# rlvc/FEALESS

Hardware: AMD Instinct MI355X
Metric: frames/sec (640x480 RGB-D x N templates, 20 ICP iters) (higher is better)
Workload: dtype u8

## Files before the change

fealess_amd/csrc/fl_context.hip:

```cpp
#include "fl_internal.h"
#include <stdlib.h>
#include <stdarg.h>
#include <string.h>
#include <algorithm>

int fl_set_error(fl_context *ctx, int code, const char *fmt, ...)
{
  if (ctx) {
    va_list ap;
    va_start(ap, fmt);
    vsnprintf(ctx->err, sizeof(ctx->err), fmt, ap);
    va_end(ap);
  }
  return code;
}

int fl_scratch(fl_context *ctx, size_t bytes, void **out)
{
  if (int rc = fl_context_join(ctx)) return rc;
  if (bytes > ctx->scratch_bytes) {
    if (ctx->scratch) {
      FL_HIP(ctx, hipStreamSynchronize(ctx->stream));
      FL_HIP(ctx, hipFree(ctx->scratch));
      ctx->scratch = nullptr;
      ctx->scratch_bytes = 0;
    }
    size_t nb = fl_align(bytes + bytes / 4, 1 << 20);
    FL_HIP(ctx, hipMalloc(&ctx->scratch, nb));
    ctx->scratch_bytes = nb;
  }
  *out = ctx->scratch;
  return FL_OK;
}

int fl_pinned(fl_context *ctx, size_t bytes, void **out)
{
  if (int rc = fl_context_join(ctx)) return rc;
  if (bytes > ctx->pinned_bytes) {
    if (ctx->pinned) {
      FL_HIP(ctx, hipStreamSynchronize(ctx->stream));
      FL_HIP(ctx, hipHostFree(ctx->pinned));
      ctx->pinned = nullptr;
      ctx->pinned_bytes = 0;
    }
    size_t nb = fl_align(bytes, 1 << 16);
    FL_HIP(ctx, hipHostMalloc(&ctx->pinned, nb, hipHostMallocDefault));
    ctx->pinned_bytes = nb;
  }
  *out = ctx->pinned;
  return FL_OK;
}

int fl_context_join(fl_context *ctx)
{
  if (!ctx->icp_pending) return FL_OK;
  ctx->icp_pending = false;
  FL_HIP(ctx, hipStreamWaitEvent(ctx->stream, ctx->ev_icp_tail, 0));
  return FL_OK;
}

int fl_context_sync_all(fl_context *ctx)
{
  FL_HIP(ctx, hipStreamSynchronize(ctx->stream));
  if (ctx->icp_stream) FL_HIP(ctx, hipStreamSynchronize(ctx->icp_stream));
  ctx->icp_pending = false;
  return FL_OK;
}

int fl_icp_stream(fl_context *ctx, hipStream_t *out)
{
  const long mode = ctx->opt.pipeline_icp;
  if (ctx->icp_stream && ctx->icp_stream_mode != mode) {
    FL_HIP(ctx, hipStreamSynchronize(ctx->icp_stream));
    FL_HIP(ctx, hipStreamDestroy(ctx->icp_stream));
    ctx->icp_stream = nullptr;
  }
  if (!ctx->icp_stream) {
    int least = 0, greatest = 0;
    FL_HIP(ctx, hipDeviceGetStreamPriorityRange(&least, &greatest));
    FL_HIP(ctx, hipStreamCreateWithPriority(&ctx->icp_stream, hipStreamNonBlocking, mode == 2 ? greatest : (mode == 3 ? least : 0)));
    ctx->icp_stream_mode = mode;
  }
  if (!ctx->ev_icp_tail) FL_HIP(ctx, hipEventCreateWithFlags(&ctx->ev_icp_tail, hipEventDisableTiming));
  *out = ctx->icp_stream;
  return FL_OK;
}

extern "C" int fl_abi_version(void) { return FL_ABI_VERSION; }

struct FlOptionName { const char *name, *env; long fl_context::Options::*field; bool hex; long lo, hi; };
static const FlOptionName fl_option_names[] = {
  {"scan_prune", "FL_SCAN_PRUNE", &fl_context::Options::scan_prune, false, 0, 1},
  {"scan_prune_mid", "FL_SCAN_PRUNE_MID", &fl_context::Options::scan_prune_mid, true, -1, 0xFF},
  {"scan_prune_lanes", "FL_SCAN_PRUNE_LANES", &fl_context::Options::scan_prune_lanes, false, 0, 1},
  {"scan_prune_step", "FL_SCAN_PRUNE_STEP", &fl_context::Options::scan_prune_step, false, 0, 8},
  {"scan_first", "FL_SCAN_FIRST", &fl_context::Options::scan_first, false, 0, 16},
  {"icp_wide", "FL_ICP_WIDE", &fl_context::Options::icp_wide, false, -1, 1},
  {"icp_occ", "FL_ICP_OCC", &fl_context::Options::icp_occ, false, 0, 5},
  {"icp_idx16", "FL_ICP_IDX16", &fl_context::Options::icp_idx16, false, -1, 1},
  {"icp_order", "FL_ICP_ORDER", &fl_context::Options::icp_order, false, 0, 1},
  {"icp_wg_per_cu", "FL_ICP_WG_PER_CU", &fl_context::Options::icp_wg_per_cu, false, 0, 3},
  {"eager_frontend", "FL_EAGER_FRONTEND", &fl_context::Options::eager_frontend, false, 0, 1},
  {"dev_poison", "FL_DEV_POISON", &fl_context::Options::dev_poison, false, 0, 1},
  {"ws_pad", "FL_DEV_WS_PAD", &fl_context::Options::ws_pad, false, 0, 16l << 20},
  {"pipeline_icp", "FL_PIPELINE_ICP", &fl_context::Options::pipeline_icp, false, 0, 3},
  {"frontend_chunk_rows", "FL_FRONTEND_CHUNK_ROWS", &fl_context::Options::frontend_chunk_rows, false, 0, 60 * 1024},
  {"scan_run", "FL_SCAN_RUN", &fl_context::Options::scan_run, false, 0, 64},
  {"refine_lds", "FL_REFINE_LDS", &fl_context::Options::refine_lds, false, 0, 2},
  {"refine_lds_bytes", "FL_REFINE_LDS_BYTES", &fl_context::Options::refine_lds_bytes, false, 0, FL_REFINE_LDS_BYTES},
  {"verify_fused", "FL_VERIFY_FUSED", &fl_context::Options::verify_fused, false, 0, 1},
  {"verify_fused_px", "FL_VERIFY_FUSED_PX", &fl_context::Options::verify_fused_px, false, 0, FL_VERIFY_FUSED_PX},
};

static bool fl_option_valid(const FlOptionName &o, long v)
{
  if (v < o.lo || v > o.hi) return false;
  if (o.field == &fl_context::Options::frontend_chunk_rows) return v % 60 == 0;
  if (o.field == &fl_context::Options::verify_fused_px) return v == 0 || v >= FL_WAVE;
  if (o.field == &fl_context::Options::scan_prune_step) return v == 0 || v == 2 || v == 4 || v == 8;
  if (o.field == &fl_context::Options::scan_first) return v == 0 || v == 8 || v == 12 || v == 14 || v == 16;
  return o.field != &fl_context::Options::icp_occ || v == 0 || v >= 4;
}

extern "C" int fl_context_create(int device, fl_context **out)
{
  if (!out) return FL_ERR_INVALID;
  *out = nullptr;
  int n = 0;
  if (hipGetDeviceCount(&n) != hipSuccess || n <= 0) return FL_ERR_NO_DEVICE;
  if (device < 0 || device >= n) return FL_ERR_INVALID;
  fl_context *ctx = new fl_context();
  ctx->device = device;
  if (hipSetDevice(device) != hipSuccess ||
      hipStreamCreateWithFlags(&ctx->own_stream, hipStreamNonBlocking) != hipSuccess) {
    delete ctx;
    return FL_ERR_HIP;
  }
  ctx->stream = ctx->own_stream;
  {
    hipDeviceProp_t prop;
    if (hipGetDeviceProperties(&prop, device) == hipSuccess && prop.multiProcessorCount > 0) ctx->cus = prop.multiProcessorCount;
  }
  for (const FlOptionName &o : fl_option_names)
    if (const char *e = getenv(o.env)) {
      const long v = o.hex ? (long)strtoul(e, nullptr, 16) : atol(e);
      if (fl_option_valid(o, v)) ctx->opt.*(o.field) = v;
    }
  *out = ctx;
  return FL_OK;
}

extern "C" void *fl_context_get_stream(fl_context *ctx) { return ctx ? (void *)ctx->stream : nullptr; }
extern "C" int fl_context_get_device(const fl_context *ctx) { return ctx ? ctx->device : -1; }
extern "C" fl_context *fl_detector_get_context(fl_detector *det) { return det ? det->ctx : nullptr; }

extern "C" int fl_context_set_option(fl_context *ctx, const char *name, long value)
{
  if (!ctx || !name) return FL_ERR_INVALID;
  for (const FlOptionName &o : fl_option_names)
    if (!strcmp(name, o.name)) {
      if (!fl_option_valid(o, value)) return fl_set_error(ctx, FL_ERR_INVALID, "option '%s': %ld is out of range", name, value);
      ctx->opt.*(o.field) = value;
      return FL_OK;
    }
  return fl_set_error(ctx, FL_ERR_INVALID, "unknown option '%s'", name);
}

extern "C" int fl_context_get_option(const fl_context *ctx, const char *name, long *value)
{
  if (!ctx || !name || !value) return FL_ERR_INVALID;
  for (const FlOptionName &o : fl_option_names)
    if (!strcmp(name, o.name)) { *value = ctx->opt.*(o.field); return FL_OK; }
  return FL_ERR_INVALID;
}

static void context_release(fl_context *ctx)
{
  if (ctx->device < 0) { delete ctx; return; }
  (void)hipSetDevice(ctx->device);
  (void)fl_context_sync_all(ctx);
  if (ctx->icp_stream) (void)hipStreamDestroy(ctx->icp_stream);
  if (ctx->ev_icp_tail) (void)hipEventDestroy(ctx->ev_icp_tail);
  if (ctx->scratch) (void)hipFree(ctx->scratch);
  if (ctx->pinned) (void)hipHostFree(ctx->pinned);
  if (ctx->own_stream) (void)hipStreamDestroy(ctx->own_stream);
  delete ctx;
}

extern "C" void fl_context_destroy(fl_context *ctx)
{
  if (!ctx) return;
  if (ctx->detectors > 0) { ctx->destroy_pending = true; return; }
  context_release(ctx);
}

extern "C" const char *fl_last_error(const fl_context *ctx) { return ctx ? ctx->err : "null context"; }

extern "C" int fl_context_set_stream(fl_context *ctx, void *hip_stream)
{
  if (!ctx) return FL_ERR_INVALID;
  if (int rc = fl_context_sync_all(ctx)) return rc;
  ctx->stream = hip_stream ? (hipStream_t)hip_stream : ctx->own_stream;
  return FL_OK;
}

extern "C" int fl_context_synchronize(fl_context *ctx)
{
  if (!ctx) return FL_ERR_INVALID;
  FL_HIP(ctx, hipSetDevice(ctx->device));
  return fl_context_sync_all(ctx);
}

extern "C" size_t fl_lm_label_stride(int w, int h, int T)
{
  size_t W = (size_t)(w / T), H = (size_t)(h / T);
  size_t pad = W * H + 16 * W + 64;
  size_t s = (size_t)T * T * W * H + pad;
  return (s + 63) & ~(size_t)63;
}

extern "C" int fl_detector_create(fl_context *ctx, int modalities, int levels, const int *T_at_level,
                                  fl_detector **out)
{
  if (!ctx || !out || !T_at_level) return FL_ERR_INVALID;
  if (modalities < 1 || modalities > FL_MAX_MODALITIES || levels < 1 || levels > FL_MAX_LEVELS)
    return fl_set_error(ctx, FL_ERR_INVALID, "modalities must be 1..%d and levels 1..%d", FL_MAX_MODALITIES,
                        FL_MAX_LEVELS);
  for (int l = 0; l < levels; ++l)
    if (T_at_level[l] < 1 || T_at_level[l] > 16) return fl_set_error(ctx, FL_ERR_INVALID, "T out of range");
  fl_detector *det = new fl_detector();
  det->ctx = ctx;
  ++ctx->detectors;
  det->M = modalities;
  det->L = levels;
  for (int l = 0; l < levels; ++l) det->T[l] = T_at_level[l];
  memset(&det->times, 0, sizeof(det->times));
  *out = det;
  return FL_OK;
}

static void free_device_tables(fl_detector *det)
{
  (void)hipFree(det->d_scan_items);
  (void)hipFree(det->d_scan_off);
  (void)hipFree(det->d_fine_hdr);
  (void)hipFree(det->d_fine_box);
  (void)hipFree(det->d_fine_feat);
  (void)hipFree(det->d_pyr);
  (void)hipFree(det->d_poses);
  (void)hipFree(det->d_class_first);
  (void)hipFree(det->d_item_enabled);
  (void)hipFree((void *)det->d_depth_ptrs);
  (void)hipFree(det->d_ws);
  (void)hipFree(det->d_results);
  if (det->h_results) (void)hipHostFree(det->h_results);
  det->d_scan_items = nullptr;
  det->n_scan_items = 0;
  det->scan_item_g.clear();
  det->d_scan_off = nullptr;
  det->d_fine_hdr = nullptr;
  det->d_fine_box = nullptr;
  det->d_fine_feat = nullptr;
  det->d_pyr = nullptr;
  det->d_poses = nullptr;
// ... 486 lines not shown
```

fealess_amd/csrc/fl_frontend.hip:

```cpp
#include "fl_internal.h"
#include <float.h>
#include <type_traits>

#ifndef FL_CQ_DOT4
#define FL_CQ_DOT4 1
#endif

__device__ __forceinline__ int clampi(int v, int lo, int hi) { return v < lo ? lo : (v > hi ? hi : v); }
__device__ __forceinline__ int reflect101(int p, int len)
{
  if (len == 1) return 0;
  while (p < 0 || p >= len) p = p < 0 ? -p : 2 * len - 2 - p;
  return p;
}

__device__ __forceinline__ float fast_atan2_deg(float y, float x)
{
  const float p1 = 0.9997878412794807f * (float)(180 / 3.14159265358979323846);
  const float p3 = -0.3258083974640975f * (float)(180 / 3.14159265358979323846);
  const float p5 = 0.1555786518463281f * (float)(180 / 3.14159265358979323846);
  const float p7 = -0.04432655554792128f * (float)(180 / 3.14159265358979323846);
  const float ax = fabsf(x), ay = fabsf(y);
  const bool steep = !(ax >= ay);
  const float c = (steep ? ax : ay) / ((steep ? ay : ax) + (float)DBL_EPSILON);
  const float c2 = c * c;
  const float poly = (((p7 * c2 + p5) * c2 + p3) * c2 + p1) * c;
  float a = steep ? 90.f - poly : poly;
  if (x < 0) a = 180.f - a;
  if (y < 0) a = 360.f - a;
  return a;
}

#define CQ_COLS 60
#define CQ_CH 60

__device__ __forceinline__ unsigned wave_from_prev(unsigned v) { return (unsigned)__builtin_amdgcn_update_dpp((int)v, (int)v, 0x138, 0xF, 0xF, false); }
__device__ __forceinline__ unsigned wave_from_next(unsigned v) { return (unsigned)__builtin_amdgcn_update_dpp((int)v, (int)v, 0x130, 0xF, 0xF, false); }
__device__ __forceinline__ unsigned wave_from_prev0(unsigned v) { return (unsigned)__builtin_amdgcn_update_dpp(0, (int)v, 0x138, 0xF, 0xF, true); }
__device__ __forceinline__ unsigned wave_from_next0(unsigned v) { return (unsigned)__builtin_amdgcn_update_dpp(0, (int)v, 0x130, 0xF, 0xF, true); }

__host__ __device__ __forceinline__ void cq_window_addr(uint32_t row_mis, int w, int xc, uint32_t *off, uint32_t *shift, int *first)
{
  const int f = xc - 3 < 0 ? 0 : (xc - 3 > w - 7 ? w - 7 : xc - 3);
  const uint32_t o = row_mis + 3u * (uint32_t)f;
  *off = o & ~3u;
  *shift = o & 3u;
  *first = f;
}

__host__ __device__ __forceinline__ uint32_t cq_alignbyte(uint32_t hi, uint32_t lo, uint32_t s)
{
#if defined(__HIP_DEVICE_COMPILE__)
  return __builtin_amdgcn_alignbyte(hi, lo, s);
#else
  return (uint32_t)((((uint64_t)hi << 32) | lo) >> (8 * (s & 3u)));
#endif
}

__host__ __device__ __forceinline__ void cq_window(const uint8_t *__restrict__ row4, uint32_t row_mis, int w, int xc, bool any_left,
                                                   bool any_right, uint32_t *wd)
{
  uint32_t off, shift;
  int first;
  cq_window_addr(row_mis, w, xc, &off, &shift, &first);
  const int dpx = xc - 3 - first;
  uint32_t d[6];
  const uint8_t *q = (const uint8_t *)__builtin_assume_aligned(row4 + off, 4);
  __builtin_memcpy(d, q, 16);
  __builtin_memcpy(d + 4, q + 16, 8);
#pragma unroll
  for (int k = 0; k < 5; ++k) wd[k] = cq_alignbyte(d[k + 1], d[k], shift);
  wd[5] = cq_alignbyte(d[5], d[5], shift);
#define CQ_TAKE(e0, e1, e2, e3, e4, e5, e6, e7, e8)                                                                                 \
  {                                                                                                                                 \
    const bool b0 = (dw & 1u) != 0u, b1 = (dw & 2u) != 0u;                                                                          \
    const uint32_t t0 = b0 ? e1 : e0, t1 = b0 ? e2 : e1, t2 = b0 ? e3 : e2, t3 = b0 ? e4 : e3, t4 = b0 ? e5 : e4, t5 = b0 ? e6 : e5, \
                   t6 = b0 ? e7 : e6, t7 = b0 ? e8 : e7;                                                                            \
    const uint32_t g0 = b1 ? t2 : t0, g1 = b1 ? t3 : t1, g2 = b1 ? t4 : t2, g3 = b1 ? t5 : t3, g4 = b1 ? t6 : t4, g5 = b1 ? t7 : t5; \
    wd[0] = cq_alignbyte(g1, g0, s);                                                                                                \
    wd[1] = cq_alignbyte(g2, g1, s);                                                                                                \
    wd[2] = cq_alignbyte(g3, g2, s);                                                                                                \
    wd[3] = cq_alignbyte(g4, g3, s);                                                                                                \
    wd[4] = cq_alignbyte(g5, g4, s);                                                                                                \
    wd[5] = cq_alignbyte(g5, g5, s);                                                                                                \
  }
  if (any_left) {
    const uint32_t s = dpx < 0 ? (uint32_t)-dpx : 0u, dw = 3u - s;
    const uint32_t p = wd[0] & 0xFFFFFFu;
    CQ_TAKE((p | (p << 24)), ((p >> 8) | (p << 16)), ((p >> 16) | (p << 8)), wd[0], wd[1], wd[2], wd[3], wd[4], wd[5])
  }
  if (any_right) {
    const uint32_t n = dpx > 0 ? 3u * (uint32_t)dpx : 0u, dw = n >> 2, s = n & 3u;
    const uint32_t p = (wd[4] >> 16) | ((wd[5] & 0xFFu) << 16);
    CQ_TAKE(wd[0], wd[1], wd[2], wd[3], wd[4], ((p >> 16) | (p << 8)), (p | (p << 24)), ((p >> 8) | (p << 16)), 0u)
  }
#undef CQ_TAKE
}

template <bool kNarrow>
__device__ __forceinline__ void cq_hrow(const uint8_t *__restrict__ src, int w, int h, int row, int xc, bool any_left, bool any_right,
                                        int *h3)
{
  const int kk[7] = {8, 28, 56, 72, 56, 28, 8};
  const uint8_t *p = src + (size_t)clampi(row, 0, h - 1) * (size_t)(w * 3);
  int a0 = 0, a1 = 0, a2 = 0;
  if (!kNarrow) {
    const uint32_t mis = (uint32_t)(uintptr_t)p & 3u;
    uint32_t wd[6];
    cq_window(p - mis, mis, w, xc, any_left, any_right, wd);
#if FL_CQ_DOT4
    unsigned acc[3] = {0u, 0u, 0u};
#pragma unroll
    for (int ch = 0; ch < 3; ++ch)
#pragma unroll
      for (int k = 0; k < 6; ++k) {
        unsigned wk = 0;
#pragma unroll
        for (int t = 0; t < 7; ++t)
          if (((3 * t + ch) >> 2) == k) wk |= (unsigned)kk[t] << (8 * ((3 * t + ch) & 3));
        if (wk != 0u) acc[ch] = __builtin_amdgcn_udot4(wd[k], wk, acc[ch], false);
      }
    a0 = (int)acc[0]; a1 = (int)acc[1]; a2 = (int)acc[2];
#else
#pragma unroll
    for (int t = 0; t < 7; ++t) {
      const int b0 = 3 * t, b1 = 3 * t + 1, b2 = 3 * t + 2;
      a0 += kk[t] * (int)((wd[b0 >> 2] >> (8 * (b0 & 3))) & 0xFFu);
      a1 += kk[t] * (int)((wd[b1 >> 2] >> (8 * (b1 & 3))) & 0xFFu);
      a2 += kk[t] * (int)((wd[b2 >> 2] >> (8 * (b2 & 3))) & 0xFFu);
    }
#endif
  } else {
#pragma unroll
    for (int t = 0; t < 7; ++t) {
      const uint8_t *q = p + 3 * clampi(xc + t - 3, 0, w - 1);
      a0 += kk[t] * q[0];
      a1 += kk[t] * q[1];
      a2 += kk[t] * q[2];
    }
  }
  h3[0] = a0;
  h3[1] = a1;
  h3[2] = a2;
}

extern "C" void fl_dev_cq_window_addr(unsigned row_mis, int w, int xc, unsigned *off, unsigned *shift, int *first)
{
  cq_window_addr(row_mis, w, xc, off, shift, first);
}
extern "C" void fl_dev_cq_window_taps(const uint8_t *row4, unsigned row_mis, int w, int xc, int any_left, int any_right, uint8_t *taps21)
{
  uint32_t wd[6];
  cq_window(row4, row_mis, w, xc, any_left != 0, any_right != 0, wd);
  for (int b = 0; b < 21; ++b) taps21[b] = (uint8_t)(wd[b >> 2] >> (8 * (b & 3)));
}

#ifndef FL_CQ_WPE
#define FL_CQ_WPE 6
#endif
template <bool kMag, bool kNarrow>
__global__ __launch_bounds__(256) __attribute__((amdgpu_waves_per_eu(kNarrow ? 6 : FL_CQ_WPE, kNarrow ? 6 : FL_CQ_WPE))) void k_color_quantize(const uint8_t *__restrict__ bgr, size_t in_stride,
                                                        uint8_t *__restrict__ dst, size_t out_stride, int w, int h,
                                                        float threshold_sq, int nstrips, int nchunks, int chunk_rows,
                                                        float *__restrict__ mag_out, const uint32_t *__restrict__ tiles,
                                                        size_t tiles_stride)
{
  const int wave = __builtin_amdgcn_readfirstlane((int)(threadIdx.x >> 6)), lane = threadIdx.x & 63;
  const int item = blockIdx.x * 4 + wave;
  if (item >= nstrips * nchunks) return;
  const int strip = item % nstrips, chunk = item / nstrips;
  int row_lo = 0, row_hi = h - 1;
  if (tiles) {
    const uint32_t *tb = tiles + (size_t)blockIdx.z * tiles_stride;
    const int t = chunk * nstrips + strip;
    if (!((tb[FL_TILE_WORDS + (t >> 5)] >> (t & 31)) & 1u)) return;
    const uint32_t rw = tb[2 * FL_TILE_WORDS + 32 * FL_TILE_WORDS + t];
    row_lo = (int)(rw >> 16);
    row_hi = (int)(rw & 0xFFFFu);
  }
  const uint8_t *src = bgr + (size_t)blockIdx.z * in_stride;
  uint8_t *out = dst + (size_t)blockIdx.z * out_stride;
  const int x = strip * CQ_COLS + lane - 2;
  const int xc = clampi(x, 0, w - 1);
  const int y0 = max(chunk * chunk_rows, row_lo), y1 = min(min(h, chunk * chunk_rows + chunk_rows), row_hi + 1);
  if (y0 >= y1) return;
  const bool any_left = strip == 0, any_right = strip * CQ_COLS + 61 > w - 4;

  int H[7][3];
  {
    const int center = clampi(y0 - 2, 0, h - 1);
#pragma unroll
    for (int i = 0; i < 7; ++i) cq_hrow<kNarrow>(src, w, h, center + i - 3, xc, any_left, any_right, H[i]);
  }
  uint32_t Sl[3] = {0, 0, 0}, Sc[3] = {0, 0, 0}, Sr[3] = {0, 0, 0};
  uint32_t Qp[3] = {0, 0, 0};
  float Mg[3] = {0.f, 0.f, 0.f};
  auto smooth = [&](int p) __attribute__((always_inline)) {
    uint32_t vv[3];
#pragma unroll
    for (int ch = 0; ch < 3; ++ch)
      vv[ch] = __umul24(8u, (unsigned)(H[p % 7][ch] + H[(p + 6) % 7][ch])) + __umul24(28u, (unsigned)(H[(p + 1) % 7][ch] + H[(p + 5) % 7][ch])) +
               __umul24(56u, (unsigned)(H[(p + 2) % 7][ch] + H[(p + 4) % 7][ch])) + __umul24(72u, (unsigned)H[(p + 3) % 7][ch]);
    const uint32_t S = (uint32_t)(((int)vv[0] + (1 << 15)) >> 16) | ((uint32_t)(((int)vv[1] + (1 << 15)) >> 16) << 8) |
                       ((uint32_t)(((int)vv[2] + (1 << 15)) >> 16) << 16);
    const uint32_t L = wave_from_prev0(S), R = wave_from_next0(S);
    Sl[0] = Sl[1]; Sl[1] = Sl[2]; Sl[2] = L;
    Sc[0] = Sc[1]; Sc[1] = Sc[2]; Sc[2] = S;
    Sr[0] = Sr[1]; Sr[1] = Sr[2]; Sr[2] = R;
  };
  auto again = [&]() __attribute__((always_inline)) {
    Sl[0] = Sl[1]; Sl[1] = Sl[2];
    Sc[0] = Sc[1]; Sc[1] = Sc[2];
    Sr[0] = Sr[1]; Sr[1] = Sr[2];
  };
  auto finish = [&](int yv) __attribute__((always_inline)) {
    if (yv < y0) return;
    const int ys = yv - 1;
    int bdx = 0, bdy = 0, bmag = 0;
    {
      int dxs[3], dys[3], mags[3];
#pragma unroll
      for (int ch = 0; ch < 3; ++ch) {
        const int sh = 8 * ch;
#define PX(v) ((int)(((v) >> sh) & 0xFFu))
        const int dx = (PX(Sr[0]) - PX(Sl[0])) + 2 * (PX(Sr[1]) - PX(Sl[1])) + (PX(Sr[2]) - PX(Sl[2]));
        const int dy = (PX(Sl[2]) - PX(Sl[0])) + 2 * (PX(Sc[2]) - PX(Sc[0])) + (PX(Sr[2]) - PX(Sr[0]));
#undef PX
        dxs[ch] = dx;
        dys[ch] = dy;
        mags[ch] = __mul24(dx, dx) + __mul24(dy, dy);
      }
      if (mags[0] >= mags[1] && mags[0] >= mags[2]) { bdx = dxs[0]; bdy = dys[0]; bmag = mags[0]; }
      else if (mags[1] >= mags[0] && mags[1] >= mags[2]) { bdx = dxs[1]; bdy = dys[1]; bmag = mags[1]; }
      else { bdx = dxs[2]; bdy = dys[2]; bmag = mags[2]; }
    }
    const float ang = fast_atan2_deg((float)bdy, (float)bdx);
    int qi = __float2int_rn(ang * (float)(16.0 / 360.0));
    qi = qi < 0 ? 0 : (qi > 255 ? 255 : qi);
    const bool inside = ys > 0 && ys < h - 1 && x > 0 && x < w - 1;
    const uint32_t q = inside ? (uint32_t)(qi & 7) : 0u;
    const uint32_t oh = 1u << (4 * q);
    const uint32_t ohl = wave_from_prev0(oh), ohr = wave_from_next0(oh);
    Qp[0] = Qp[1]; Qp[1] = Qp[2]; Qp[2] = oh + ohl + ohr;
    Mg[0] = Mg[1]; Mg[1] = Mg[2]; Mg[2] = (float)bmag;
    if (yv < y0 + 2) return;
    const int yo = yv - 2;
    if (lane >= 2 && lane < 2 + CQ_COLS && x < w && yo < y1) {
      uint8_t res = 0;
      if (yo >= 1 && yo < h - 1 && x >= 1 && x < w - 1 && Mg[1] > threshold_sq) {
        const unsigned hist = Qp[0] + Qp[1] + Qp[2];
        const unsigned maj = (hist + 0x33333333u) & 0x88888888u;
        if (maj) res = (uint8_t)(1u << ((__ffs((int)maj) - 4) >> 2));
      }
      out[(size_t)yo * w + x] = res;
      if (kMag) mag_out[(size_t)blockIdx.z * out_stride + (size_t)yo * w + x] = Mg[1];
      else if (mag_out) mag_out[(size_t)yo * w + x] = Mg[1];
    }
  };

  const int ylast = y1 + 1, yadv = min(ylast, h - 1);
  int yv = y0 - 2;
  smooth(0);
  for (++yv; yv <= min(ylast, 0); ++yv) {
    again();
    finish(yv);
  }
  for (;;) {
#pragma unroll
    for (int P = 0; P < 7; ++P) {
      if (yv > yadv) goto below;
      cq_hrow<kNarrow>(src, w, h, yv + 3, xc, any_left, any_right, H[P]);
      smooth(P + 1);
      finish(yv);
      ++yv;
    }
  }
below:
  for (; yv <= ylast; ++yv) {
    again();
    finish(yv);
  }
}

int fl_launch_quantized_orientations(fl_context *ctx, const uint8_t *bgr, size_t in_stride, uint8_t *dst,
                                     size_t out_stride, int n_frames, int w, int h, float weak_threshold)
{
  return fl_launch_quantized_orientations_mag(ctx, bgr, in_stride, dst, out_stride, n_frames, w, h, weak_threshold, nullptr);
}

#define FL_CHUNK_FILL 4
template <typename K>
static long waves_per_cu(K kernel, long *cache)
{
  if (*cache == 0) {
    int blocks = 0;
    *cache = hipOccupancyMaxActiveBlocksPerMultiprocessor(&blocks, kernel, 256, 0) == hipSuccess && blocks > 0 ? 4l * blocks : 32;
  }
  return *cache;
}
static int fl_eager_chunk_rows(const fl_context *ctx, long per_cu, int nstrips, int n_frames, int h)
{
  if (ctx->opt.frontend_chunk_rows) return (int)ctx->opt.frontend_chunk_rows;
  const long need = (long)FL_CHUNK_FILL * ctx->cus * per_cu;
  return h > 60 && (long)nstrips * n_frames * ((h + 119) / 120) >= need ? 120 : 60;
}

static_assert(CQ_COLS == FL_TILE && CQ_CH == FL_TILE, "the lazy tile grid is k_color_quantize's work decomposition");
static int launch_color_quantize(fl_context *ctx, const uint8_t *bgr, size_t in_stride, uint8_t *dst, size_t out_stride, int n_frames,
                                 int w, int h, float weak_threshold, float *mag_out, const uint32_t *tiles, size_t tiles_stride)
{
  static long per_cu[4] = {0, 0, 0, 0};
  const int nstrips = (w + CQ_COLS - 1) / CQ_COLS;
  const bool narrow = w < 8;
  auto launch = [&](auto kernel, long *cache) {
    const int rows = tiles ? CQ_CH : fl_eager_chunk_rows(ctx, waves_per_cu(kernel, cache), nstrips, n_frames, h);
    const int nchunks = (h + rows - 1) / rows;
    dim3 grid((nstrips * nchunks + 3) / 4, 1, n_frames);
    hipLaunchKernelGGL(kernel, grid, dim3(256), 0, ctx->stream, bgr, in_stride, dst, out_stride, w, h, weak_threshold * weak_threshold,
                       nstrips, nchunks, rows, mag_out, tiles, tiles_stride);
  };
  if (mag_out) {
    if (narrow) launch(k_color_quantize<true, true>, &per_cu[3]);
    else launch(k_color_quantize<true, false>, &per_cu[1]);
  } else {
    if (narrow) launch(k_color_quantize<false, true>, &per_cu[2]);
    else launch(k_color_quantize<false, false>, &per_cu[0]);
  }
  FL_HIP(ctx, hipGetLastError());
  return FL_OK;
}

int fl_launch_quantized_orientations_mag(fl_context *ctx, const uint8_t *bgr, size_t in_stride, uint8_t *dst,
                                         size_t out_stride, int n_frames, int w, int h, float weak_threshold, float *mag_out)
{
  return launch_color_quantize(ctx, bgr, in_stride, dst, out_stride, n_frames, w, h, weak_threshold, mag_out, nullptr, 0);
}

__device__ __forceinline__ void pyrdown_general_px(const uint8_t *__restrict__ src, int w, int h, int x, int y, uint8_t *o)
{
  const int k[5] = {1, 4, 6, 4, 1};
  int acc0 = 0, acc1 = 0, acc2 = 0;
#pragma unroll
  for (int j = 0; j < 5; ++j) {
    const int yy = reflect101(2 * y + j - 2, h);
    int r0 = 0, r1 = 0, r2 = 0;
#pragma unroll
    for (int i = 0; i < 5; ++i) {
      const int xx = reflect101(2 * x + i - 2, w);
      const uint8_t *p = src + ((size_t)yy * w + xx) * 3;
      r0 += k[i] * p[0];
      r1 += k[i] * p[1];
      r2 += k[i] * p[2];
    }
    acc0 += k[j] * r0;
    acc1 += k[j] * r1;
    acc2 += k[j] * r2;
  }
  o[0] = (uint8_t)((acc0 + 128) >> 8);
  o[1] = (uint8_t)((acc1 + 128) >> 8);
  o[2] = (uint8_t)((acc2 + 128) >> 8);
}

__global__ __launch_bounds__(256) void k_pyrdown_general(const uint8_t *__restrict__ src_, size_t in_stride,
                                                         uint8_t *__restrict__ dst_, size_t out_stride, int w, int h)
{
  const int dw = w / 2, dh = h / 2;
  const int x = blockIdx.x * 32 + (threadIdx.x & 31), y = blockIdx.y * 8 + (threadIdx.x >> 5);
  if (x >= dw || y >= dh) return;
  const uint8_t *src = src_ + (size_t)blockIdx.z * in_stride;
  uint8_t *dst = dst_ + (size_t)blockIdx.z * out_stride;
  pyrdown_general_px(src, w, h, x, y, dst + ((size_t)y * dw + x) * 3);
}

#define PD_ROWS 8
__global__ __launch_bounds__(256) void k_pyrdown_pairs(const uint8_t *__restrict__ src_, size_t in_stride,
                                                       uint8_t *__restrict__ dst_, size_t out_stride, int w, int h)
{
  const int dw = w / 2, dh = h / 2, np = dw / 2;
  const int per = (np + (int)gridDim.x - 1) / (int)gridDim.x, lane = threadIdx.x & 63;
  const int xp = blockIdx.x * per + lane;
  const int y0 = (blockIdx.y * 4 + (threadIdx.x >> 6)) * PD_ROWS;
  if (lane >= per || xp >= np || y0 >= dh) return;
  const uint8_t *src = src_ + (size_t)blockIdx.z * in_stride;
  uint8_t *dst = dst_ + (size_t)blockIdx.z * out_stride;
  const bool first = xp == 0, last = xp == np - 1;
  const bool wave_first = blockIdx.x == 0, wave_last = blockIdx.x == gridDim.x - 1;
  const int off16 = first ? 0 : 12 * xp - 8, off8 = first ? 16 : (last ? 12 * xp + 4 : 12 * xp + 8);
  auto hrow = [&](int r, int (&o)[6]) {
    const int yy = reflect101(r, h);
    uint32_t wd[6];
    const uint8_t *p = src + (size_t)yy * w * 3;
    __builtin_memcpy(wd, p + off16, 16);
    __builtin_memcpy(wd + 4, p + off8, 8);
    if (wave_first) {
      const uint32_t mix = (wd[2] & 0xFFu) | ((wd[0] >> 24) << 8) | (wd[1] << 16);
      const uint32_t n0 = wd[1], n2 = wd[0], n3 = wd[1], n4 = wd[2], n5 = wd[3];
      wd[0] = first ? n0 : wd[0];
      wd[1] = first ? mix : wd[1];
      wd[2] = first ? n2 : wd[2];
      wd[3] = first ? n3 : wd[3];
      wd[4] = first ? n4 : wd[4];
      wd[5] = first ? n5 : wd[5];
    }
    if (wave_last) {
      const uint32_t hi = wd[5];
      wd[4] = last ? hi : wd[4];
      wd[5] = last ? ((wd[3] >> 16) | (hi << 16)) : wd[5];
    }
#define SB(b) ((int)((wd[(b) >> 2] >> (8 * ((b) & 3))) & 0xFFu))
#pragma unroll
    for (int ch = 0; ch < 3; ++ch) {
      o[ch] = SB(2 + ch) + 4 * SB(5 + ch) + 6 * SB(8 + ch) + 4 * SB(11 + ch) + SB(14 + ch);
      o[3 + ch] = SB(8 + ch) + 4 * SB(11 + ch) + 6 * SB(14 + ch) + 4 * SB(17 + ch) + SB(20 + ch);
    }
#undef SB
  };
  int H[5][6];
  hrow(2 * y0 - 2, H[0]);
  hrow(2 * y0 - 1, H[1]);
  hrow(2 * y0, H[2]);
#pragma unroll
  for (int k = 0; k < PD_ROWS; ++k) {
    const int y = y0 + k;
    if (y < dh) {
      hrow(2 * y + 1, H[(2 * k + 3) % 5]);
      hrow(2 * y + 2, H[(2 * k + 4) % 5]);
      uint32_t v[6];
#pragma unroll
      for (int c = 0; c < 6; ++c) {
        const int acc = H[(2 * k) % 5][c] + 4 * H[(2 * k + 1) % 5][c] + 6 * H[(2 * k + 2) % 5][c] + 4 * H[(2 * k + 3) % 5][c] +
                        H[(2 * k + 4) % 5][c];
        v[c] = (uint32_t)((acc + 128) >> 8);
      }
      uint16_t *o = (uint16_t *)(dst + ((size_t)y * dw + 2 * xp) * 3);
      o[0] = (uint16_t)(v[0] | (v[1] << 8));
      o[1] = (uint16_t)(v[2] | (v[3] << 8));
      o[2] = (uint16_t)(v[4] | (v[5] << 8));
    }
  }
}

int fl_launch_pyrdown_bgr(fl_context *ctx, const uint8_t *src, size_t in_stride, uint8_t *dst, size_t out_stride,
                          int n_frames, int w, int h)
{
  const int dw = w / 2, dh = h / 2;
  const bool pairs_ok = dw >= 8 && (w & 1) == 0 && (dw & 1) == 0 && ((3 * dw) & 1) == 0 && (out_stride & 1) == 0 && (((size_t)dst) & 1) == 0;
  if (!pairs_ok) {
    dim3 grid((dw + 31) / 32, (dh + 7) / 8, n_frames);
    hipLaunchKernelGGL(k_pyrdown_general, grid, dim3(256), 0, ctx->stream, src, in_stride, dst, out_stride, w, h);
  } else {
    dim3 grid((dw / 2 + 63) / 64, (dh + 4 * PD_ROWS - 1) / (4 * PD_ROWS), n_frames);
    hipLaunchKernelGGL(k_pyrdown_pairs, grid, dim3(256), 0, ctx->stream, src, in_stride, dst, out_stride, w, h);
  }
  FL_HIP(ctx, hipGetLastError());
  return FL_OK;
}

__constant__ uint8_t c_normal_lut[400];
static bool g_normal_lut_ready[64] = {false};

static int ensure_normal_lut(fl_context *ctx)
{
  if (ctx->device < 64 && g_normal_lut_ready[ctx->device]) return FL_OK;
  uint8_t lut[400];
  for (int y = 0; y < 20; ++y)
    for (int x = 0; x < 20; ++x) {
      double best = -1e300;
      int bk = 0;
      for (int k = 0; k < 8; ++k) {
        double a = k * (3.14159265358979323846 / 4);
        double d = (x - 10) * cos(a) + (y - 10) * sin(a);
        if (d > best + 1e-9) { best = d; bk = k; }
      }
      lut[y * 20 + x] = (uint8_t)(1 << bk);
    }
  FL_HIP(ctx, hipMemcpyToSymbol(HIP_SYMBOL(c_normal_lut), lut, sizeof(lut)));
  if (ctx->device < 64) g_normal_lut_ready[ctx->device] = true;
  return FL_OK;
}

#define DQ_COLS 60
// ... 472 lines not shown
```

fealess_amd/csrc/fl_internal.h:

```cpp
#pragma once
#include <hip/hip_runtime.h>
#include <cmath>
#include <stdint.h>
#include <stdio.h>
#include <string>
#include <vector>
#include "../../include/fealess_hip.h"

#define FL_WAVE 64

struct fl_context {
  int device = 0;
  hipStream_t own_stream = nullptr;
  hipStream_t stream = nullptr;
  hipStream_t icp_stream = nullptr;
  long icp_stream_mode = 0;
  hipEvent_t ev_icp_tail = nullptr;
  bool icp_pending = false;
  char err[512] = {0};
  void *scratch = nullptr;
  size_t scratch_bytes = 0;
  void *pinned = nullptr;
  size_t pinned_bytes = 0;
  int cus = 256;
  struct Options {
    long scan_prune = 1;
    long scan_prune_mid = -1;
    long scan_prune_lanes = 1;
    long scan_prune_step = 0;
    long scan_first = 0;
    long icp_wide = -1;
    long icp_occ = 0;
    long icp_idx16 = -1;
    long icp_order = 1;
    long icp_wg_per_cu = 0;
    long eager_frontend = 0;
    long dev_poison = 0;
    long ws_pad = 0;
    long pipeline_icp = 3;
    long frontend_chunk_rows = 0;
    long scan_run = 0;
    long refine_lds = 0;
    long refine_lds_bytes = 0;
    long verify_fused = 0;
    long verify_fused_px = 0;
  } opt;
  bool verify_fused_attr = false;
  int detectors = 0;
  bool destroy_pending = false;
};

int fl_set_error(fl_context *ctx, int code, const char *fmt, ...);
int fl_scratch(fl_context *ctx, size_t bytes, void **out);
int fl_pinned(fl_context *ctx, size_t bytes, void **out);
int fl_context_join(fl_context *ctx);
int fl_context_sync_all(fl_context *ctx);
int fl_icp_stream(fl_context *ctx, hipStream_t *out);

#define FL_HIP(ctx, call)                                                                  \
  do {                                                                                     \
    hipError_t e_ = (call);                                                                \
    if (e_ != hipSuccess)                                                                  \
      return fl_set_error((ctx), FL_ERR_HIP, "%s:%d: %s -> %s", __FILE__, __LINE__, #call, \
                          hipGetErrorString(e_));                                          \
  } while (0)

static inline size_t fl_align(size_t v, size_t a) { return (v + a - 1) / a * a; }
static inline bool fl_finite_all(const float *p, size_t n)
{
  for (size_t i = 0; i < n; ++i)
    if (!std::isfinite(p[i])) return false;
  return true;
}

#define FL_MAX_LEVELS 4
#define FL_MAX_MODALITIES 2
#define FL_MAX_FEATURES 63

struct FlScanHdr {
  int32_t P;
  int32_t off_begin;
  int32_t n_pad;
  int32_t nf;
};
struct FlScanItem {
  uint32_t off0[8];
  int32_t g;
  uint32_t chunk_nf;
  struct {
    int32_t P;
    int32_t off_begin;
    uint32_t npad_nf;
  } mod[FL_MAX_MODALITIES];
};
static_assert(sizeof(FlScanItem) == 64 && FL_MAX_MODALITIES == 2, "a dword per lane of a 16-lane load");
#define FL_SCAN_OFF_PAD 8
void fl_build_scan_items(const std::vector<FlScanHdr> &hdr, int n_pyr, int M, int WH, uint32_t zero_off, std::vector<uint32_t> &scan_off,
                         std::vector<FlScanItem> &items);
struct FlFineFeat {
  int16_t x, y;
  int16_t qx, qy;
  uint8_t gx, gy;
  uint8_t label, pad;
};
struct FlFineHdr {
  int32_t feat_begin, feat_count;
  int32_t width, height;
};
struct FlFineBox {
  int16_t x0, y0, x1, y1;
};
struct FlPyrInfo {
  int32_t class_idx, template_id;
  int32_t off_x0, off_y0, width0, height0;
  int32_t depth_slot;
  int32_t pad;
};
struct FlCand {
  int32_t x, y;
  int32_t g;
  float sim;
};

struct FlRefineJob {
  int32_t frame;
  fl_match match;
};

#define FL_REFINE_LDS_BYTES 65536
#define FL_REFINE_GROUP_MAX 8
#define FL_REFINE_BLOCK 256
struct FlRect { int x0, y0, x1, y1; };
__host__ __device__ inline int fl_refine_pitch(int width, uint32_t qmask)
{
  int q = (width + 3) >> 2;
  while (!((qmask >> (q & 31)) & 1u)) ++q;
  return q * 4;
}
__host__ __device__ inline uint32_t fl_refine_qmask(int T)
{
  uint32_t mask = 0;
  int best = 33;
  for (int q = 0; q < 32; q += 4) {
    int n[32] = {0}, worst = 0;
    for (int row = 0; row < 8; ++row)
      for (int cg = 0; cg < 4; ++cg) {
        const int b = (T * (row * q + cg)) & 31;
        if (++n[b] > worst) worst = n[b];
      }
    if (worst < best) { best = worst; mask = 0; }
    if (worst == best) mask |= 1u << q;
  }
  return mask;
}
__host__ __device__ inline FlRect fl_rect_union(FlRect a, FlRect b)
{
  if (a.x1 < a.x0) return b;
  if (b.x1 < b.x0) return a;
  FlRect r;
  r.x0 = a.x0 < b.x0 ? a.x0 : b.x0;
  r.y0 = a.y0 < b.y0 ? a.y0 : b.y0;
  r.x1 = a.x1 > b.x1 ? a.x1 : b.x1;
  r.y1 = a.y1 > b.y1 ? a.y1 : b.y1;
  return r;
}
__host__ __device__ inline long fl_refine_window_bytes(FlRect r, uint32_t qmask)
{
  if (r.x1 < r.x0) return 0;
  return (long)fl_refine_pitch(r.x1 - (r.x0 & ~3) + 1, qmask) * (r.y1 - r.y0 + 1);
}
template <typename C>
__host__ __device__ inline int fl_refine_plan(const C *rects, int n, int max_len, long budget, uint32_t qmask, FlRect *uni)
{
  FlRect u = {rects[0], rects[1], rects[2], rects[3]};
  int len = 1;
  while (len < n && len < max_len) {
    const C *c = rects + 4 * len;
    const FlRect r = {c[0], c[1], c[2], c[3]};
    const FlRect v = fl_rect_union(u, r);
    if (fl_refine_window_bytes(v, qmask) > budget) break;
    u = v;
    ++len;
  }
  *uni = u;
  return len;
}
extern "C" int fl_dev_refine_pitch(int width, int T);
extern "C" int fl_dev_refine_plan(const int32_t *rects, int n, int max_len, long budget, int T, int32_t *uni);
extern "C" int fl_dev_refine_kernel(const fl_detector *det, int level);
extern "C" long fl_dev_refine_window_max(const fl_detector *det, int level);

#define FL_TILE 60
#define FL_TILE_WORDS 16
#define FL_TILE_BLOCK_WORDS (66 * FL_TILE_WORDS)
#define FL_NUM_EVENTS 24

struct FlLevelGeom {
  int32_t w, h, T, W, H, WH;
// ... 261 lines not shown
```

Before: 92960.

## Skip orientation labelling for strip rows with no strong-magnitude pixels

Adds a wave ballot marking pixels whose gradient magnitude exceeds the weak threshold. The atan2 quantisation and neighbour one-hot exchange are computed only when a three-row window holds such pixels, and the output stage is shifted by one row to make room. Output and magnitude stores now go through incrementally advanced row pointers with opaque lane offsets. This is meant to cut ALU and cross-lane work on flat image regions, at the cost of extra pipeline state, one more closing iteration, and some risk of edge-case mismatches at strip or row borders. An optional compile-time stats counter is also added.

```diff
diff --git a/fealess_amd/csrc/fl_context.hip b/fealess_amd/csrc/fl_context.hip
--- a/fealess_amd/csrc/fl_context.hip
+++ b/fealess_amd/csrc/fl_context.hip
@@ -110,6 +110,7 @@
   {"refine_lds_bytes", "FL_REFINE_LDS_BYTES", &fl_context::Options::refine_lds_bytes, false, 0, FL_REFINE_LDS_BYTES},
   {"verify_fused", "FL_VERIFY_FUSED", &fl_context::Options::verify_fused, false, 0, 1},
   {"verify_fused_px", "FL_VERIFY_FUSED_PX", &fl_context::Options::verify_fused_px, false, 0, FL_VERIFY_FUSED_PX},
+  {"cq_label_skip", "FL_CQ_LABEL_SKIP", &fl_context::Options::cq_label_skip, false, 0, 1},
 };
 
 static bool fl_option_valid(const FlOptionName &o, long v)
diff --git a/fealess_amd/csrc/fl_frontend.hip b/fealess_amd/csrc/fl_frontend.hip
--- a/fealess_amd/csrc/fl_frontend.hip
+++ b/fealess_amd/csrc/fl_frontend.hip
@@ -158,12 +158,15 @@
 #ifndef FL_CQ_WPE
 #define FL_CQ_WPE 6
 #endif
+#ifdef FL_CQ_STATS
+__device__ unsigned long long d_cq_stats[2];
+#endif
 template <bool kMag, bool kNarrow>
 __global__ __launch_bounds__(256) __attribute__((amdgpu_waves_per_eu(kNarrow ? 6 : FL_CQ_WPE, kNarrow ? 6 : FL_CQ_WPE))) void k_color_quantize(const uint8_t *__restrict__ bgr, size_t in_stride,
                                                         uint8_t *__restrict__ dst, size_t out_stride, int w, int h,
                                                         float threshold_sq, int nstrips, int nchunks, int chunk_rows,
                                                         float *__restrict__ mag_out, const uint32_t *__restrict__ tiles,
-                                                        size_t tiles_stride)
+                                                        size_t tiles_stride, float strong_sq)
 {
   const int wave = __builtin_amdgcn_readfirstlane((int)(threadIdx.x >> 6)), lane = threadIdx.x & 63;
   const int item = blockIdx.x * 4 + wave;
@@ -213,11 +216,20 @@
     Sc[0] = Sc[1]; Sc[1] = Sc[2];
     Sr[0] = Sr[1]; Sr[1] = Sr[2];
   };
-  auto finish = [&](int yv) __attribute__((always_inline)) {
+  unsigned ox = (unsigned)x, ox4 = 4u * (unsigned)x;
+  auto lane_off = [](unsigned &off) __attribute__((always_inline)) { asm volatile("" : "+v"(off)); return off; };
+  uint8_t *orow = out + (size_t)y0 * (size_t)w;
+  float *mrow = kMag ? mag_out + (size_t)blockIdx.z * out_stride + (size_t)y0 * (size_t)w : (mag_out ? mag_out + (size_t)y0 * (size_t)w : nullptr);
+  int pdx = 0, pdy = 0;
+  unsigned sf0 = 0, sf1 = 0, sf2 = 0;
+#ifdef FL_CQ_STATS
+  unsigned st_rows = 0, st_labelled = 0;
+#endif
+  auto finish = [&](int yv, bool closing) __attribute__((always_inline)) {
     if (yv < y0) return;
-    const int ys = yv - 1;
     int bdx = 0, bdy = 0, bmag = 0;
-    {
+    unsigned long long strong = 0;
+    if (!closing) {
       int dxs[3], dys[3], mags[3];
 #pragma unroll
       for (int ch = 0; ch < 3; ++ch) {
@@ -233,29 +245,49 @@
       if (mags[0] >= mags[1] && mags[0] >= mags[2]) { bdx = dxs[0]; bdy = dys[0]; bmag = mags[0]; }
       else if (mags[1] >= mags[0] && mags[1] >= mags[2]) { bdx = dxs[1]; bdy = dys[1]; bmag = mags[1]; }
       else { bdx = dxs[2]; bdy = dys[2]; bmag = mags[2]; }
-    }
-    const float ang = fast_atan2_deg((float)bdy, (float)bdx);
-    int qi = __float2int_rn(ang * (float)(16.0 / 360.0));
-    qi = qi < 0 ? 0 : (qi > 255 ? 255 : qi);
-    const bool inside = ys > 0 && ys < h - 1 && x > 0 && x < w - 1;
-    const uint32_t q = inside ? (uint32_t)(qi & 7) : 0u;
-    const uint32_t oh = 1u << (4 * q);
-    const uint32_t ohl = wave_from_prev0(oh), ohr = wave_from_next0(oh);
-    Qp[0] = Qp[1]; Qp[1] = Qp[2]; Qp[2] = oh + ohl + ohr;
+      strong = __builtin_amdgcn_ballot_w64((float)bmag > strong_sq) & 0x3FFFFFFFFFFFFFFCull;
+    }
     Mg[0] = Mg[1]; Mg[1] = Mg[2]; Mg[2] = (float)bmag;
-    if (yv < y0 + 2) return;
-    const int yo = yv - 2;
-    if (lane >= 2 && lane < 2 + CQ_COLS && x < w && yo < y1) {
-      uint8_t res = 0;
-      if (yo >= 1 && yo < h - 1 && x >= 1 && x < w - 1 && Mg[1] > threshold_sq) {
+    sf0 = sf1; sf1 = sf2; sf2 = (unsigned)strong | (unsigned)(strong >> 32);
+    const bool label = (sf0 | sf1 | sf2) != 0u;
+    const int yl = yv - 2;
+    uint32_t rowsum = 0;
+    if (label) {
+      const float ang = fast_atan2_deg((float)pdy, (float)pdx);
+      int qi = __float2int_rn(ang * (float)(16.0 / 360.0));
+      qi = qi < 0 ? 0 : (qi > 255 ? 255 : qi);
+      const bool inside = yl > 0 && yl < h - 1 && x > 0 && x < w - 1;
+      const uint32_t q = inside ? (uint32_t)(qi & 7) : 0u;
+      const uint32_t oh = 1u << (4 * q);
+      const uint32_t ohl = wave_from_prev0(oh), ohr = wave_from_next0(oh);
+      rowsum = oh + ohl + ohr;
+    }
+#ifdef FL_CQ_STATS
+    if (yl >= y0 && yl < y1) {
+      ++st_rows;
+      if (label) ++st_labelled;
+    }
+#endif
+    Qp[0] = Qp[1]; Qp[1] = Qp[2]; Qp[2] = rowsum;
+    pdx = bdx;
+    pdy = bdy;
+    if (yv < y0 + 3) return;
+    const int yo = yv - 3;
+    uint8_t res = 0;
+    if (sf0 != 0u && yo >= 1 && yo < h - 1) {
+      if (x >= 1 && x < w - 1 && Mg[0] > threshold_sq) {
+        asm volatile("");
         const unsigned hist = Qp[0] + Qp[1] + Qp[2];
         const unsigned maj = (hist + 0x33333333u) & 0x88888888u;
         if (maj) res = (uint8_t)(1u << ((__ffs((int)maj) - 4) >> 2));
       }
-      out[(size_t)yo * w + x] = res;
-      if (kMag) mag_out[(size_t)blockIdx.z * out_stride + (size_t)yo * w + x] = Mg[1];
-      else if (mag_out) mag_out[(size_t)yo * w + x] = Mg[1];
-    }
+    }
+    if (lane >= 2 && lane < 2 + CQ_COLS && x < w && yo < y1) {
+      orow[lane_off(ox)] = res;
+      if (kMag || mrow) *(float *)((char *)mrow + lane_off(ox4)) = Mg[0];
+    }
+    orow += w;
+    if (kMag || mrow) mrow += w;
   };
 
   const int ylast = y1 + 1, yadv = min(ylast, h - 1);
@@ -263,7 +295,7 @@
   smooth(0);
   for (++yv; yv <= min(ylast, 0); ++yv) {
     again();
-    finish(yv);
+    finish(yv, false);
   }
   for (;;) {
 #pragma unroll
@@ -271,15 +303,21 @@
       if (yv > yadv) goto below;
       cq_hrow<kNarrow>(src, w, h, yv + 3, xc, any_left, any_right, H[P]);
       smooth(P + 1);
-      finish(yv);
+      finish(yv, false);
       ++yv;
     }
   }
 below:
-  for (; yv <= ylast; ++yv) {
+  for (; yv <= ylast + 1; ++yv) {
     again();
-    finish(yv);
-  }
+    finish(yv, yv > ylast);
+  }
+#ifdef FL_CQ_STATS
+  if (lane == 0) {
+    atomicAdd(&d_cq_stats[0], (unsigned long long)st_rows);
+    atomicAdd(&d_cq_stats[1], (unsigned long long)st_labelled);
+  }
+#endif
 }
 
 int fl_launch_quantized_orientations(fl_context *ctx, const uint8_t *bgr, size_t in_stride, uint8_t *dst,
@@ -316,8 +354,9 @@
     const int rows = tiles ? CQ_CH : fl_eager_chunk_rows(ctx, waves_per_cu(kernel, cache), nstrips, n_frames, h);
     const int nchunks = (h + rows - 1) / rows;
     dim3 grid((nstrips * nchunks + 3) / 4, 1, n_frames);
-    hipLaunchKernelGGL(kernel, grid, dim3(256), 0, ctx->stream, bgr, in_stride, dst, out_stride, w, h, weak_threshold * weak_threshold,
-                       nstrips, nchunks, rows, mag_out, tiles, tiles_stride);
+    const float threshold_sq = weak_threshold * weak_threshold;
+    hipLaunchKernelGGL(kernel, grid, dim3(256), 0, ctx->stream, bgr, in_stride, dst, out_stride, w, h, threshold_sq, nstrips, nchunks,
+                       rows, mag_out, tiles, tiles_stride, ctx->opt.cq_label_skip ? threshold_sq : -1.f);
   };
   if (mag_out) {
     if (narrow) launch(k_color_quantize<true, true>, &per_cu[3]);
@@ -327,6 +366,16 @@
     else launch(k_color_quantize<false, false>, &per_cu[0]);
   }
   FL_HIP(ctx, hipGetLastError());
+#ifdef FL_CQ_STATS
+  {
+    unsigned long long st[2], zero[2] = {0, 0};
+    FL_HIP(ctx, hipStreamSynchronize(ctx->stream));
+    FL_HIP(ctx, hipMemcpyFromSymbol(st, HIP_SYMBOL(d_cq_stats), sizeof(st)));
+    FL_HIP(ctx, hipMemcpyToSymbol(HIP_SYMBOL(d_cq_stats), zero, sizeof(zero)));
+    fprintf(stderr, "k_color_quantize: %d frames %dx%d%s, %llu strip rows walked, %llu labelled (%.1f %%)\n", n_frames, w, h,
+            tiles ? " (tiles)" : "", st[0], st[1], st[0] ? 100.0 * (double)st[1] / (double)st[0] : 0.0);
+  }
+#endif
   return FL_OK;
 }
 
diff --git a/fealess_amd/csrc/fl_internal.h b/fealess_amd/csrc/fl_internal.h
--- a/fealess_amd/csrc/fl_internal.h
+++ b/fealess_amd/csrc/fl_internal.h
@@ -44,6 +44,7 @@
     long refine_lds_bytes = 0;
     long verify_fused = 0;
     long verify_fused_px = 0;
+    long cq_label_skip = 1;
   } opt;
   bool verify_fused_attr = false;
   int detectors = 0;
```

After: 93840 (median of 6 runs). No clear change (+0.9%).
